# mastbaum/sxmc

Hardware: AMD Instinct MI355X
Metric: NLL evals/sec (10^8 samples, 3 obs, 12 signals) + experiments/sec at 1/2/4/8 GPUs (higher is better)
Workload: dtype f64 exact; f32-on-u16-codes filter decides the unambiguous samples

## Files before the change

### sxmc_amd/csrc/fill_kernels.inc.h

```cpp
#pragma once

#include "sxmc_device_types.h"

#pragma clang fp contract(off)

#ifndef SXMC_MEASURE
#define SXMC_MEASURE 0
#endif

namespace sxfill {

__device__ __forceinline__ constexpr unsigned sx_dbg(unsigned dbg_arg) { return SXMC_MEASURE ? dbg_arg : 0u; }

template <int N>
struct IntC {
  static constexpr int value = N;
  constexpr operator int() const { return N; }
};
template <unsigned long... I>
struct ISeq {};
template <int N, unsigned long... I>
struct MakeISeq : MakeISeq<N - 1, (unsigned long)(N - 1), I...> {};
template <unsigned long... I>
struct MakeISeq<0, I...> {
// ... 107 lines not shown
        pw[q] = 1.0;
        pl[q] = 0.0;
      }
      for (int i = 0; i < npars; i++) {
        const double c = readlane_d(coef, cstart + i);
#pragma unroll
        for (int q = 0; q < SXMC_VEC; q++) {
          p[q] = p[q] + c * pw[q];
          pow_step(pw[q], pl[q], f[K][q]);
        }
      }
    }
    apply_transform<NSLOT>(f, type, f[K], extra_slot, p);
  });
}

constexpr unsigned sx_op(int type, int obs_slot, int extra_slot = 0, int npars = 0) {
  return (unsigned)type | ((unsigned)obs_slot << 4) | ((unsigned)extra_slot << 8) | ((unsigned)npars << 12);
}
constexpr int sx_op_npars(unsigned w) { return ((w >> 12) & 15u) ? (int)((w >> 12) & 15u) : 1; }
template <unsigned... OPS>
constexpr int sx_prog_ncoef() {
  constexpr unsigned ops[] = {OPS..., 0u};
  int c = 0;
  for (int k = 0; k < (int)sizeof...(OPS); k++) c += sx_op_npars(ops[k]);
  return c;
}
template <unsigned... OPS>
constexpr int sx_prog_cstart(int i) {
  constexpr unsigned ops[] = {OPS..., 0u};
  int c = 0;
  for (int k = 0; k < i; k++) c += sx_op_npars(ops[k]);
  return c;
}
template <unsigned... OPS>
struct StaticProg {
  static constexpr bool dynamic = false;
  static constexpr int n = (int)sizeof...(OPS);
  static constexpr int ncoef = sx_prog_ncoef<OPS...>();
  static constexpr unsigned touched = (0u | ... | (1u << ((OPS >> 4) & 15u)));
};
struct DynamicProg {
  static constexpr bool dynamic = true;
  static constexpr int n = 0;
  static constexpr int ncoef = 0;
  static constexpr unsigned touched = ~0u;
};

template <int NSLOT, unsigned OPC>
__device__ __forceinline__ void apply_static(double (&f)[NSLOT][SXMC_VEC], const double* c) {
  constexpr int type = (int)(OPC & 15u), K = (int)((OPC >> 4) & 15u), E = (int)((OPC >> 8) & 15u);
  constexpr int NP = sx_op_npars(OPC);
  static_assert(K < NSLOT && E < NSLOT, "slot out of range");
#pragma unroll
  for (int q = 0; q < SXMC_VEC; q++) {
    double pc = 0.0 + c[0] * 1.0;
    if constexpr (NP > 1) {
      double pw = 1.0 * f[K][q], pl = 0.0;
#pragma unroll
      for (int i = 1; i < NP; i++) {
        pc = pc + c[i] * pw;
        pow_step(pw, pl, f[K][q]);
      }
    }
    if constexpr (type == SXMC_SYST_SHIFT) f[K][q] = f[K][q] + pc;
    if constexpr (type == SXMC_SYST_SCALE) f[K][q] = f[K][q] * (1 + pc);
    if constexpr (type == SXMC_SYST_CTSCALE) f[K][q] = 1 + (f[K][q] - 1) * (1 + pc);
    if constexpr (type == SXMC_SYST_RESOLUTION_SCALE) f[K][q] = f[K][q] + (pc * (f[K][q] - f[E][q]));
  }
}

template <int NSLOT, unsigned... OPS, unsigned long... I>
__device__ __forceinline__ void run_static(double (&f)[NSLOT][SXMC_VEC], const double* c, StaticProg<OPS...>,
                                           ISeq<I...>) {
  (apply_static<NSLOT, OPS>(f, c + sx_prog_cstart<OPS...>((int)I)), ...);
}

typedef float vfloat4 __attribute__((ext_vector_type(4)));

#ifndef SXMC_WG_STAMPS
#define SXMC_WG_STAMPS 0
#endif
#if SXMC_WG_STAMPS && !defined(__HIPCC_RTC__)
extern "C" __device__ unsigned long long sx_wg_stamps[3 * 4096];
#define SX_WG_STAMP(which)                                                                      \
  do {                                                                                          \
    if (threadIdx.x == 0 && blockIdx.x < 4096u) {                                               \
      sx_wg_stamps[(which)*4096 + blockIdx.x] = __builtin_amdgcn_s_memrealtime();               \
    }                                                                                           \
  } while (0)
#else
#define SX_WG_STAMP(which) \
  do {                     \
  } while (0)
#endif
#ifndef SXMC_CACHED_LOADS
#define SXMC_CACHED_LOADS 0
#endif
template <typename T>
__device__ __forceinline__ T stream_load(gptr<const T> p) {
  if constexpr (SXMC_CACHED_LOADS) return *p;
  else return __builtin_nontemporal_load(p);
}

typedef unsigned vuint2 __attribute__((ext_vector_type(2)));

__device__ __forceinline__ void sparse_lookup(const SxSignalDesc& d, gptr<unsigned> counters, unsigned bin) {
  const unsigned mask = (1u << (32 - d.sparse_table_shift)) - 1u;
  unsigned hp = (bin * 0x85EBCA6Bu) >> d.sparse_table_shift;
  for (unsigned probe = 0; probe <= mask; probe++) {
    const vuint2 e = to_global(reinterpret_cast<const vuint2*>(d.sparse_table))[hp];
    if (e[0] == bin) {
      __hip_atomic_fetch_add(&counters[e[1]], 1u, __ATOMIC_RELAXED, __HIP_MEMORY_SCOPE_AGENT);
      return;
    }
    if (e[0] == 0xFFFFFFFFu) return;
    hp = (hp + 1u) & mask;
  }
}

__device__ __forceinline__ void sparse_count(const SxSignalDesc& d, gptr<unsigned> counters, unsigned bin) {
  const unsigned hb = (bin * 0x9E3779B1u) >> d.sparse_filter_shift;
  if (!((to_global(d.sparse_filter)[hb >> 5] >> (hb & 31u)) & 1u)) return;
  sparse_lookup(d, counters, bin);
}

constexpr int kPreGranule = 3;
template <int PREW> struct PreVec { typedef unsigned type; };
template <> struct PreVec<2> { typedef unsigned type __attribute__((ext_vector_type(2))); };
template <> struct PreVec<4> { typedef unsigned type __attribute__((ext_vector_type(4))); };

template <int NSLOT, int PREW>
struct Columns {
  vfloat4 v[NSLOT];
  typename PreVec<PREW>::type pre;
};

template <int NOBS, int PREW, typename PROG>
constexpr bool slot_loaded(int k) {
  return PREW == 0 || PREW == kPreGranule || k >= NOBS || ((PROG::touched >> k) & 1u);
}

template <int PREW>
__device__ __forceinline__ unsigned pre_value(const typename PreVec<PREW>::type& p, int q) {
  if constexpr (PREW == 1) return (p >> (8 * q)) & 0xFFu;
  if constexpr (PREW == 2) return (p[q >> 1] >> (16 * (q & 1))) & 0xFFFFu;
  if constexpr (PREW == 4) return p[q];
  if constexpr (PREW == kPreGranule) return p;
  return 0u;
}
template <int PREW>
constexpr unsigned pre_sentinel() {
  return PREW == 1 ? 0xFFu : PREW == 2 ? 0xFFFFu : 0xFFFFFFFFu;
}

template <int NOBS, int NSLOT, int PREW, typename PROG>
__device__ __forceinline__ void load_columns(Columns<NSLOT, PREW>& c, const gptr<const vfloat4> (&col)[NSLOT],
                                             gptr<const typename PreVec<PREW>::type> pre, unsigned long long v) {
#pragma unroll
  for (int k = 0; k < NSLOT; k++) {
    if constexpr (true) {
      if (slot_loaded<NOBS, PREW, PROG>(k)) {
        c.v[k] = stream_load<vfloat4>(&col[k][v]);
        __builtin_amdgcn_sched_barrier(0);
      }
    }
  }
  if constexpr (PREW == kPreGranule) {
    c.pre = pre[v >> 6];
    __builtin_amdgcn_sched_barrier(0);
  } else if constexpr (PREW != 0) {
    c.pre = stream_load<typename PreVec<PREW>::type>(&pre[v]);
    __builtin_amdgcn_sched_barrier(0);
  }
}

// ... 1483 lines not shown
        unsigned n = 0u;
        for (unsigned r = 0; r < R; r++) n += hist[(unsigned)c * cstride + r * rstride + w];
        total += n;
        if (n != 0u) __hip_atomic_fetch_add(&gbins[lds_slot(w)], n, __ATOMIC_RELAXED, __HIP_MEMORY_SCOPE_AGENT);
      }
      if (use_q) {
#pragma unroll
        for (int off = kWave / 2; off > 0; off >>= 1) total += __shfl_down(total, off, kWave);
        if (lane == 0 && total != 0u) {
          __hip_atomic_fetch_add(&s_norm[c], total, __ATOMIC_RELAXED, __HIP_MEMORY_SCOPE_WORKGROUP);
        }
        __syncthreads();
      }
      if (LDS_HIST && more) {
        __syncthreads();
        for (unsigned b = 4u * tid; b < cstride; b += 4u * nthreads) {
          *reinterpret_cast<vuint4g*>(&hist[(unsigned)c * cstride + b]) = vuint4g{0u, 0u, 0u, 0u};
        }
      }
      if (tid == 0) {
        const unsigned n = s_norm[c];
        if (n != 0u) __hip_atomic_fetch_add(to_global(dc.norm), n, __ATOMIC_RELAXED, __HIP_MEMORY_SCOPE_AGENT);
        s_norm[c] = 0u;
      }
    }
    __syncthreads();
    lds_clean = true;
  }
  SX_WG_STAMP(2);
}

template <unsigned OPC, int XT>
__device__ __forceinline__ void apply_box_interval(double& xl, double& xh, double tl, double th, bool& fin, const double* c) {
  constexpr int type = (int)(OPC & 15u), E = (int)((OPC >> 8) & 15u);
  static_assert(sx_op_npars(OPC) == 1, "not a one-coefficient systematic");
  const double pc = 0.0 + c[0] * 1.0;
  if constexpr (type == SXMC_SYST_SHIFT) {
    xl = xl + pc;
    xh = xh + pc;
  }
  if constexpr (type == SXMC_SYST_SCALE) {
    const double s = 1 + pc, a = xl * s, b = xh * s;
    xl = s >= 0.0 ? a : b;
    xh = s >= 0.0 ? b : a;
  }
  if constexpr (type == SXMC_SYST_CTSCALE) {
    const double s = 1 + pc, a = 1 + (xl - 1) * s, b = 1 + (xh - 1) * s;
    xl = s >= 0.0 ? a : b;
    xh = s >= 0.0 ? b : a;
  }
  if constexpr (type == SXMC_SYST_RESOLUTION_SCALE) {
    static_assert(E == XT, "the boxed observable reads one truth field");
    const double dl = xl - th, dh = xh - tl;
    const double a = pc * dl, b = pc * dh;
    const double ml = pc >= 0.0 ? a : b, mh = pc >= 0.0 ? b : a;
    fin = fin && (__builtin_fabs(dl) < __builtin_inf()) && (__builtin_fabs(dh) < __builtin_inf()) &&
          (__builtin_fabs(ml) < __builtin_inf()) && (__builtin_fabs(mh) < __builtin_inf());
    xl = xl + ml;
    xh = xh + mh;
  }
  fin = fin && (__builtin_fabs(xl) < __builtin_inf()) && (__builtin_fabs(xh) < __builtin_inf());
}
template <int BX, int XT, unsigned... OPS, unsigned long... I>
__device__ __forceinline__ void run_box_interval(double& xl, double& xh, double tl, double th, bool& fin, const double* c,
                                                 StaticProg<OPS...>, ISeq<I...>) {
  ([&] {
    if constexpr ((int)((OPS >> 4) & 15u) == BX) apply_box_interval<OPS, XT>(xl, xh, tl, th, fin, c + sx_prog_cstart<OPS...>((int)I));
  }(), ...);
}
template <int BX, int XT, unsigned... OPS>
constexpr bool prog_is_boxable(StaticProg<OPS...>) {
  return (true && ... &&
          (sx_op_npars(OPS) == 1 && (int)((OPS >> 4) & 15u) != XT &&
           ((int)(OPS & 15u) != SXMC_SYST_RESOLUTION_SCALE ||
            ((int)((OPS >> 4) & 15u) == BX && (int)((OPS >> 8) & 15u) == XT))));
}

#ifndef SXMC_BOX_DRAIN
#define SXMC_BOX_DRAIN 2
#endif
#ifndef SXMC_BOX_GQ
#define SXMC_BOX_GQ 0
#endif
#ifndef SXMC_BOX_PREFETCH
#define SXMC_BOX_PREFETCH 0
#endif
template <int NOBS, int NSLOT, typename PROG>
__device__ __forceinline__ void fill_boxed_body(const SxSignalDesc* __restrict__ descs, const SxSegment* __restrict__ segs,
                                                const unsigned* __restrict__ blk_off, unsigned layout, unsigned dbg_arg) {
  const unsigned dbg = sx_dbg(dbg_arg);
  static_assert(!PROG::dynamic && NOBS == 1 && NSLOT == 3, "one streamed observable, one truth field, the boxed observable");
  constexpr int BX = 2, XT = 1;
  static_assert(prog_is_boxable<BX, XT>(PROG{}), "not a program the boxed form can run");
  constexpr int NC = PROG::ncoef > 0 ? PROG::ncoef : 1;
#ifndef SXMC_BOX_RING
#define SXMC_BOX_RING 8
#endif
  constexpr int kRing = SXMC_BOX_RING;
  constexpr int kDrain = SXMC_BOX_DRAIN;
  static_assert(64 % kRing == 0, "a block of 64 units is a whole number of rounds of the ring");
  typedef typename MakeISeq<PROG::n>::type Seq;
  extern __shared__ unsigned lds[];
  const unsigned tid = threadIdx.x;
  const unsigned nthreads = blockDim.x;
  const unsigned lane = tid & (kWave - 1);
  unsigned* s_norm = lds;
  unsigned* hist = lds + 4;
  const unsigned rstride = layout & 0xFFFFFFu, rlog = (layout >> 24) & 7u, R = 1u << rlog;
  const unsigned cstride = rstride << rlog;
  const unsigned myrep = (lane & (R - 1u)) * rstride;
  const unsigned qlog = layout >> 28;
  const unsigned qwave = qlog ? (1u << qlog) / (nthreads / kWave) : 0u;
  const unsigned gq_min = (unsigned)kRing + 1u;
  const unsigned gq_cap = qwave / 2u > gq_min ? qwave / 2u : gq_min, rq_cap = qwave > gq_cap ? qwave - gq_cap : 0u;
  const unsigned gq_drain = (SXMC_BOX_GQ > 0 && (unsigned)SXMC_BOX_GQ + (unsigned)kRing < gq_cap) ? (unsigned)SXMC_BOX_GQ + (unsigned)kRing : gq_cap;
  unsigned* qrows = lds + 4 + cstride + 64 + 4 + (tid / kWave) * (2u * qwave);
  unsigned* qgran = qrows + 2u * rq_cap;

  bool lds_clean = false;
  const unsigned seg_end = blk_off[blockIdx.x + 1];
  for (unsigned si = blk_off[blockIdx.x]; si < seg_end; ++si) {
    const SxSegment& sg = segs[si];
    const SxSignalDesc& d = descs[sg.sig];
    const unsigned long long v0 = sg.v0, v1 = sg.v1, step = sg.step;
    const unsigned B = (unsigned)d.total_nbins;
    double craw[NC];
#pragma unroll
    for (int q = 0; q < PROG::ncoef; q++) craw[q] = to_global(d.params)[(long)d.coef_par[q] * d.param_stride];
    __builtin_amdgcn_sched_barrier(0);

    gptr<const vfloat4> col[NSLOT];
#pragma unroll
    for (int k = 0; k < NSLOT; k++) {
      col[k] = to_global(reinterpret_cast<const vfloat4*>(d.cols + (unsigned long long)d.slot_col[k] * d.col_pitch));
    }
    gptr<const unsigned> precol = to_global(reinterpret_cast<const unsigned*>(d.pre));
    gptr<const vfloat4> boxes = to_global(reinterpret_cast<const vfloat4*>(d.boxes));
    gptr<const vuint2g> qcol = to_global(d.qcol != nullptr ? reinterpret_cast<const vuint2g*>(d.qcol)
                                                           : reinterpret_cast<const vuint2g*>(d.cols));
    const unsigned vfirst32 = (unsigned)(v0 + tid), step32 = (unsigned)step, vlast32 = (unsigned)(v1 - 1);
    const unsigned vwave32 = vfirst32 - lane;
    const unsigned niter32 = (unsigned)((v1 - v0 + step - 1) / step);

    if (!lds_clean) {
      for (unsigned b = tid; b < cstride; b += nthreads) hist[b] = 0u;
      if (tid < 4) s_norm[tid] = 0u;
      __syncthreads();
    }

    const double lo = d.lower[0], hi = d.upper[0], sc = d.scale[0];
    const int st = d.bin_stride[0];
    const unsigned nbk = (unsigned)d.nbins[0];
    const double olo = d.lower[NOBS], ohi = d.upper[NOBS], osc = d.scale[NOBS];
    const int ost = d.bin_stride[NOBS];
    int stv = st, ostv = ost;
    asm volatile("" : "+v"(stv));
    asm volatile("" : "+v"(ostv));
    const unsigned s_in = (unsigned)st, s_out = s_in * nbk;
    const unsigned oS = B / nbk, oSp = oS | 1u;
    const float inv_in = 1.0f / (float)s_in, inv_out = 1.0f / (float)s_out;
    auto fdiv = [](unsigned x, float inv) -> unsigned { return (unsigned)(((float)x + 0.5f) * inv); };
    auto hist_word = [&](unsigned bin) -> unsigned {
      const unsigned h = fdiv(bin, inv_out), rem = bin - h * s_out, idx = fdiv(rem, inv_in);
      return (idx + 1u) * oSp + h * s_in + (rem - idx * s_in);
    };

    bool wild = false;
#pragma unroll
    for (int q = 0; q < PROG::ncoef; q++) wild = wild || !(__builtin_fabs(craw[q]) < __builtin_inf());

    float af, gf, thr;
    bool use_q = d.qcol != nullptr && rq_cap >= 8u && !wild;
    {
      AffineForm<1> form[1];
      form[0].a[0] = 1.0;
      form[0].c = 0.0;
      const double wlo = d.qbase[0], whi = d.qbase[0] + 65534.0 * d.qstep[0];
      form[0].mag = __builtin_fmax(__builtin_fabs(wlo), __builtin_fabs(whi));
      run_affine<1, BX>(form, craw, PROG{}, Seq{});
      const double alpha = form[0].a[0] * d.qstep[0] * sc;
      const double sum_abs = __builtin_fabs(alpha);
      double g = form[0].c - lo;
      g = g + form[0].a[0] * (d.qbase[0] + 0.5 * d.qstep[0]);
      g = g * sc;
      const double mu = sum_abs * 65536.0 + __builtin_fabs(g) + (double)nbk + 0.25;
      const double epsq = 0.5 * sum_abs * (1.0 + 0x1p-19);
      const double eps = epsq + mu * 0x1p-21 + (form[0].mag + __builtin_fabs(lo)) * sc * 0x1p-44;
      const bool ok = eps < 0.125;
      const double e = eps * 1.01, slack = 0x1p-23;
      af = uniform_f((float)alpha);
      gf = uniform_f((float)(g + e));
      thr = uniform_f((float)(2.0 * e + slack));
      use_q = use_q && (uniform_i(ok ? 1 : 0) != 0);
    }

    unsigned vcnt = 0u;
    unsigned nrow = 0u, ngran = 0u;

    unsigned gword = kOrdSkip, greal = 0u;
    vfloat4 bx_next;
    unsigned pre_next;
    auto meta_load = [&](unsigned it) {
      unsigned vg = vwave32 + (it + lane) * step32;
      vg = vg <= vlast32 ? vg : vlast32;
      bx_next = boxes[vg >> 6];
      pre_next = precol[vg >> 6];
    };
    auto granule_meta = [&](unsigned it) {
      unsigned vg = vwave32 + (it + lane) * step32;
      const bool live = vg <= vlast32;
      vg = live ? vg : vlast32;
      if constexpr (!SXMC_BOX_PREFETCH) meta_load(it);
      const vfloat4 bx = bx_next;
      const unsigned pre = pre_next;
      if constexpr (SXMC_BOX_PREFETCH) meta_load(it + 64u);
      double xl = (double)bx.x, xh = (double)bx.y;
      const double tl = (double)bx.z, th = (double)bx.w;
      bool fin = (__builtin_fabs(xl) < __builtin_inf()) && (__builtin_fabs(xh) < __builtin_inf()) &&
                 (__builtin_fabs(tl) < __builtin_inf()) && (__builtin_fabs(th) < __builtin_inf());
      run_box_interval<BX, XT>(xl, xh, tl, th, fin, craw, PROG{}, Seq{});
      const int i0 = (int)((xl - olo) * osc), i1 = (int)((xh - olo) * osc);
      const int e0 = !(xl >= olo) ? -1 : (!(xl < ohi) ? 0x7FFFFFFF : i0);
      const int e1 = !(xh >= olo) ? -1 : (!(xh < ohi) ? 0x7FFFFFFF : i1);
      const unsigned off = (pre & 0xFFFFFFu) + (unsigned)e0 * (unsigned)ost;
      const unsigned h = fdiv(off, inv_out), rem = off - h * s_out;
      const bool canon = off < (1u << 22) && rem < s_in && (h + 1u) * s_out <= B;
      const bool mixed = !use_q || !fin || e0 != e1 || !canon;
      const bool skip = fin && e0 == e1 && (e0 < 0 || e0 == 0x7FFFFFFF);
      gword = !live ? kOrdSkip : skip ? kOrdSkip : mixed ? kOrdMixed : h * s_in + rem;
      greal = off;
    };

    auto push_granule = [&](unsigned it) {
      if (lane == 0) qgran[2u * ngran] = vwave32 + it * step32;
      ngran += 1u;
    };
    auto push_rows = [&](unsigned rare, unsigned v, unsigned real_off) -> bool {
      unsigned long long mask[SXMC_VEC];
      unsigned total = 0u;
#pragma unroll
      for (int q = 0; q < SXMC_VEC; q++) {
        mask[q] = __builtin_amdgcn_ballot_w64(((rare >> q) & 1u) != 0u);
        total += (unsigned)__builtin_popcountll(mask[q]);
      }
      if (nrow + total > rq_cap) return false;
#pragma unroll
      for (int q = 0; q < SXMC_VEC; q++) {
        if (mask[q] == 0ull) continue;
        const unsigned below = __builtin_amdgcn_mbcnt_hi((unsigned)(mask[q] >> 32),
                                                         __builtin_amdgcn_mbcnt_lo((unsigned)mask[q], 0u));
        if ((rare >> q) & 1u) {
          const unsigned pos = nrow + below;
          qrows[2u * pos] = v * SXMC_VEC + (unsigned)q;
          qrows[2u * pos + 1u] = real_off;
        }
        nrow += (unsigned)__builtin_popcountll(mask[q]);
      }
      return true;
    };

    const int oS4 = (int)(4u * oSp);
    const int oclamp = (dbg & 4u) ? -1 : (int)nbk;
    auto coarse_unit = [&](const vuint2g& w, unsigned it, unsigned v, unsigned word0) {
      int base4 = (int)(4u * (4u + myrep + word0) + 4u * oSp);
      asm volatile("" : "+v"(base4));
      const float c0 = (float)(w.x & 0xFFFFu), c1 = (float)(w.x >> 16), c2 = (float)(w.y & 0xFFFFu), c3 = (float)(w.y >> 16);
      const vfloat2 a2 = {af, af}, g2 = {gf, gf};
      const vfloat2 u01 = __builtin_elementwise_fma(a2, vfloat2{c0, c1}, g2);
      const vfloat2 u23 = __builtin_elementwise_fma(a2, vfloat2{c2, c3}, g2);
      const float us[SXMC_VEC] = {u01.x, u01.y, u23.x, u23.y};
      int addr[SXMC_VEC];
      bool amb[SXMC_VEC];
#pragma unroll
      for (int q = 0; q < SXMC_VEC; q++) {
        const float u = us[q];
        amb[q] = !(__builtin_amdgcn_fractf(u) >= thr);
        int idx;
        asm("v_cvt_flr_i32_f32 %0, %1" : "=v"(idx) : "v"(u));
        int ie;
        asm("v_med3_i32 %0, %1, -1, %2" : "=v"(ie) : "v"(amb[q] ? -1 : idx), "s"(oclamp));
        addr[q] = mad24(ie, oS4, base4);
      }
      const float cmax = __builtin_fmaxf(__builtin_fmaxf(c0, c1), __builtin_fmaxf(c2, c3));
      const bool special = cmax >= (float)SXMC_QCODE_EXACT;
      const bool anyamb = (amb[0] | amb[1]) | (amb[2] | amb[3]);
      if (__builtin_amdgcn_ballot_w64(anyamb || special) != 0ull) {
        const float cs[SXMC_VEC] = {c0, c1, c2, c3};
        unsigned rare = 0u;
#pragma unroll
        for (int q = 0; q < SXMC_VEC; q++) {
          rare |= amb[q] ? (1u << q) : 0u;
          if (cs[q] >= (float)SXMC_QCODE_EXACT) {
            addr[q] = base4 - oS4;
            rare = cs[q] >= (float)SXMC_QCODE_NEVER ? (rare & ~(1u << q)) : (rare | (1u << q));
          }
        }
        const unsigned real_off = (unsigned)__builtin_amdgcn_readlane((int)greal, (int)(it & 63u));
        if (!push_rows(rare, v, real_off)) {
          push_granule(it);
          return;
        }
      }
      if (dbg & 32u) {
        vcnt += (unsigned)(addr[0] ^ addr[1] ^ addr[2] ^ addr[3]) == 12345u ? 1u : 0u;
        return;
      }
#pragma unroll
      for (int q = 0; q < SXMC_VEC; q++) {
        unsigned* wp = reinterpret_cast<unsigned*>(reinterpret_cast<char*>(lds) + addr[q]);
        __hip_atomic_fetch_add(wp, 1u, __ATOMIC_RELAXED, __HIP_MEMORY_SCOPE_WORKGROUP);
      }
    };

    auto count_exact = [&](bool ind, int bin) {
      vcnt += (ind && !((unsigned)bin < B)) ? 1u : 0u;
      if (ind && ((unsigned)bin < B)) {
        __hip_atomic_fetch_add(&hist[myrep + hist_word((unsigned)bin)], 1u, __ATOMIC_RELAXED, __HIP_MEMORY_SCOPE_WORKGROUP);
      }
    };
    auto drain = [&]() {
      if (dbg & 16u) nrow = ngran = 0u;
      vfloat4 rawf[kDrain][NSLOT];
      unsigned prew[kDrain];
      auto load_granule = [&](int s, unsigned g) {
        const unsigned vw = (unsigned)uniform_i((int)qgran[2u * g]);
        const unsigned vc = vw + lane < vlast32 ? vw + lane : vlast32;
#pragma unroll
        for (int k = 0; k < NSLOT; k++) rawf[s][k] = __builtin_nontemporal_load(&col[k][vc]);
        prew[s] = precol[vc >> 6];
      };
      unsigned row = 0u, w1 = 0u;
      float rowf = 0.0f;
      if (lane < nrow) {
        row = qrows[2u * lane];
        w1 = qrows[2u * lane + 1u];
        rowf = ((gptr<const float>)col[0])[row];
      }
#pragma unroll
      for (int s = 0; s < kDrain; s++) {
        if ((unsigned)s < ngran) load_granule(s, (unsigned)s);
      }
      for (unsigned i0 = 0; i0 < nrow; i0 += kWave) {
        if (i0 != 0u && i0 + lane < nrow) {
          row = qrows[2u * (i0 + lane)];
          w1 = qrows[2u * (i0 + lane) + 1u];
          rowf = ((gptr<const float>)col[0])[row];
        }
        if (i0 + lane < nrow) {
          double f[NSLOT][SXMC_VEC];
#pragma unroll
          for (int k = 0; k < NSLOT; k++) f[k][0] = f[k][1] = f[k][2] = f[k][3] = 0.0;
          f[0][0] = f[0][1] = f[0][2] = f[0][3] = (double)rowf;
          run_static_part<NSLOT, BX, false>(f, craw, PROG{}, Seq{});
          const double x = f[0][0];
          const bool ind = (x >= lo) & (x < hi);
          const int idx = (int)((x - lo) * sc);
          count_exact(ind, mad24(idx, stv, (int)w1));
        }
      }
      for (unsigned g0 = 0; g0 < ngran; g0 += (unsigned)kDrain) {
        if (g0 != 0u) {
#pragma unroll
          for (int s = 0; s < kDrain; s++) {
            if (g0 + (unsigned)s < ngran) load_granule(s, g0 + (unsigned)s);
          }
        }
#pragma unroll
        for (int s = 0; s < kDrain; s++) {
          if (g0 + (unsigned)s >= ngran) break;
          const unsigned off = (unsigned)uniform_i((int)prew[s]) & 0xFFFFFFu;
          double f[NSLOT][SXMC_VEC];
#pragma unroll
          for (int k = 0; k < NSLOT; k++) {
            f[k][0] = (double)rawf[s][k].x;
            f[k][1] = (double)rawf[s][k].y;
            f[k][2] = (double)rawf[s][k].z;
            f[k][3] = (double)rawf[s][k].w;
          }
          run_static<NSLOT>(f, craw, PROG{}, Seq{});
#pragma unroll
          for (int q = 0; q < SXMC_VEC; q++) {
            const double x = f[0][q], y = f[BX][q];
            const bool ind = (x >= lo) & (x < hi) & (y >= olo) & (y < ohi);
            const int idx = (int)((x - lo) * sc), oidx = (int)((y - olo) * osc);
            count_exact(ind, mad24(oidx, ostv, mad24(idx, stv, (int)off)));
          }
        }
      }
      nrow = ngran = 0u;
    };

    vuint2g rq[kRing];
    const unsigned vfirst8 = vfirst32 * 8u, vlast8 = vlast32 * 8u, step8 = step32 * 8u;
    auto issue = [&](int slot, unsigned it) {
      unsigned o = vfirst8 + it * step8;
      o = o < vlast8 ? o : vlast8;
      rq[slot] = __builtin_nontemporal_load((gptr<const vuint2g>)((gptr<const char>)qcol + (unsigned long long)o));
      __builtin_amdgcn_sched_barrier(0);
    };
    const unsigned climit = (unsigned)uniform_i((int)oS);
    {
      unsigned it = 0u;
      if constexpr (SXMC_BOX_PREFETCH) meta_load(0u);
#pragma unroll
      for (int i = 0; i < kRing; i++) issue(i, (unsigned)i);
      while (it < niter32) {
        if ((it & 63u) == 0u) granule_meta(it);
        const unsigned block_end = niter32 < (it | 63u) + 1u ? niter32 : (it | 63u) + 1u;
        bool full = false;
        while (it < block_end && !full) {
#pragma unroll
          for (int i = 0; i < kRing; i++) {
#pragma unroll
            for (int e = 0; e < 2; e++) asm volatile("" : "+v"(rq[i][e]));
            const unsigned iu = it + (unsigned)i;
            if (iu < block_end) {
              const unsigned word0 = (unsigned)__builtin_amdgcn_readlane((int)gword, (int)(iu & 63u));
              if (dbg & 1u) {
                vcnt += (rq[i].x == 12345u && word0 == 77u) ? 1u : 0u;
              } else if (word0 < climit) coarse_unit(rq[i], iu, vfirst32 + iu * step32, word0);
              else if (word0 == kOrdMixed) push_granule(iu);
            }
            issue(i, iu + (unsigned)kRing);
          }
          it = block_end - it < (unsigned)kRing ? block_end : it + (unsigned)kRing;
          full = ngran + (unsigned)kRing > gq_drain;
        }
        if (full) {
          drain();
          __builtin_amdgcn_s_waitcnt(0);
        }
      }
    }
    drain();

    {
      unsigned t = vcnt;
#pragma unroll
      for (int off = kWave / 2; off > 0; off >>= 1) t += __shfl_down(t, off, kWave);
      if (lane == 0 && t != 0u) __hip_atomic_fetch_add(&s_norm[0], t, __ATOMIC_RELAXED, __HIP_MEMORY_SCOPE_WORKGROUP);
    }
    __syncthreads();
    {
      gptr<unsigned> gbins = to_global(d.bins);
      const bool more = si + 1u < seg_end;
      const unsigned nwords = nbk * oSp;
      const float invSp = 1.0f / (float)oSp;
      unsigned total = 0u;
#pragma unroll 4
      for (unsigned w = tid; w < nwords; w += nthreads) {
        const unsigned idx = fdiv(w, invSp), r = w - idx * oSp;
        unsigned n = 0u;
        for (unsigned rep = 0; rep < R; rep++) n += hist[rep * rstride + oSp + w];
        if (r < oS) {
          total += n;
          const unsigned h = fdiv(r, inv_in);
          if (n != 0u) {
            __hip_atomic_fetch_add(&gbins[h * s_out + idx * s_in + (r - h * s_in)], n, __ATOMIC_RELAXED, __HIP_MEMORY_SCOPE_AGENT);
          }
        }
      }
#pragma unroll
      for (int off = kWave / 2; off > 0; off >>= 1) total += __shfl_down(total, off, kWave);
      if (lane == 0 && total != 0u) __hip_atomic_fetch_add(&s_norm[0], total, __ATOMIC_RELAXED, __HIP_MEMORY_SCOPE_WORKGROUP);
      __syncthreads();
      if (more) {
        for (unsigned b = 4u * tid; b < cstride; b += 4u * nthreads) {
          *reinterpret_cast<vuint4g*>(&hist[b]) = vuint4g{0u, 0u, 0u, 0u};
        }
      }
      if (tid == 0) {
        const unsigned n = s_norm[0];
        if (n != 0u) __hip_atomic_fetch_add(to_global(d.norm), n, __ATOMIC_RELAXED, __HIP_MEMORY_SCOPE_AGENT);
        s_norm[0] = 0u;
      }
    }
    __syncthreads();
    lds_clean = true;
  }
}

template <int NOBS, int NSLOT, bool LDS_HIST, typename PROG, int PREW>
__global__ __launch_bounds__(1024) void fill_kernel(const SxSignalDesc* __restrict__ descs,
                                                    const SxSegment* __restrict__ segs,
                                                    const unsigned* __restrict__ blk_off, unsigned hist_words,
                                                    unsigned dbg) {
  fill_body<NOBS, NSLOT, LDS_HIST, PROG, PREW>(descs, segs, blk_off, hist_words, dbg);
}

template <int NOBS, int NSLOT, typename PROG>
__global__ __launch_bounds__(1024) void fill_sparse_kernel(const SxSignalDesc* __restrict__ descs,
                                                           const SxSegment* __restrict__ segs,
                                                           const unsigned* __restrict__ blk_off, unsigned smax,
                                                           unsigned dbg) {
  fill_sparse_body<NOBS, NSLOT, PROG>(descs, segs, blk_off, smax, dbg);
}

#ifndef SXMC_ORDERED_BOUND
#define SXMC_ORDERED_BOUND 1024
#endif
template <int NOBS, int NSLOT, typename PROG, bool LDS_HIST = true>
__global__ __launch_bounds__(SXMC_ORDERED_BOUND) void fill_ordered_kernel(const SxSignalDesc* __restrict__ descs,
                                                            const SxSegment* __restrict__ segs,
                                                            const unsigned* __restrict__ blk_off, unsigned layout,
                                                            unsigned dbg) {
  SxChainDescs one;
  one.d[0] = one.d[1] = one.d[2] = one.d[3] = descs;
  fill_ordered_body<NOBS, NSLOT, PROG, 1, LDS_HIST>(one, segs, blk_off, layout, dbg);
}

template <int NOBS, int NSLOT, typename PROG>
__global__ __launch_bounds__(SXMC_ORDERED_BOUND) void fill_boxed_kernel(const SxSignalDesc* __restrict__ descs,
                                                          const SxSegment* __restrict__ segs,
                                                          const unsigned* __restrict__ blk_off, unsigned layout,
                                                          unsigned dbg) {
  fill_boxed_body<NOBS, NSLOT, PROG>(descs, segs, blk_off, layout, dbg);
}

}
```

### sxmc_amd/csrc/pdfz_kernels.hip

```cpp
#include <hip/hip_runtime.h>
#include <hip/hip_ext.h>

#include <cstring>
#include <vector>

#include "nll_device.h"

#include "fill_kernels.inc.h"

#pragma clang fp contract(off)

namespace {

using namespace sxfill;


__global__ __launch_bounds__(256) void zero_kernel(const SxSignalDesc* __restrict__ descs, unsigned* ticket) {
  const SxSignalDesc& d = descs[blockIdx.y];
  unsigned* bins = d.bins;
  const unsigned n = (unsigned)d.total_nbins;
  const unsigned n4 = n >> 2;
  uint4* b4 = reinterpret_cast<uint4*>(bins);
  const unsigned stride = gridDim.x * blockDim.x;
  for (unsigned i = blockIdx.x * blockDim.x + threadIdx.x; i < n4; i += stride) {
// ... 640 lines not shown
      sxdev::peek_next_proposal_device(a.nparameters, a.rng, a.jump_width, a.v_current, v_b);
    } else {
      collect();
    }
    __syncthreads();
    for (int j = threadIdx.x; j < nsig; j += blockDim.x) {
      *hist_a[j].norm = 0u;
      *hist_b[j].norm = 0u;
    }
    return;
  }
  const bool second = blockIdx.x >= nvb;
  const unsigned vb = second ? blockIdx.x - nvb : blockIdx.x;
  const double t = eval_nll_block_part(second ? lookup_b : lookup_a, nsig, npoints, second ? weight_b : weight_a,
                                       second ? v_b : a.v_proposed, a.nexpected, a.n_mc, a.source_id,
                                       second ? norms_b : a.norms, sh, vb, nvb);
  __shared__ int s_clear;
  if (threadIdx.x == 0) {
    __hip_atomic_store(slots + blockIdx.x, isnan(t) ? kSlotNaN : (unsigned long long)__double_as_longlong(t),
                       __ATOMIC_RELAXED, __HIP_MEMORY_SCOPE_AGENT);
    asm volatile("s_waitcnt vmcnt(0)" ::: "memory");
    unsigned it = 0;
    for (; it < kEndSpinLimit; it++) {
      if (__hip_atomic_load(slots + blockIdx.x, __ATOMIC_RELAXED, __HIP_MEMORY_SCOPE_AGENT) == kSlotEmpty) break;
      __builtin_amdgcn_s_sleep(1);
    }
    if (it == kEndSpinLimit) __hip_atomic_fetch_add(timeouts, 1u, __ATOMIC_RELAXED, __HIP_MEMORY_SCOPE_AGENT);
    s_clear = it < kEndSpinLimit ? 1 : 0;
  }
  __syncthreads();
  if (!s_clear) return;
  const unsigned npieces = 2u * zblocks * (unsigned)nsig;
  for (unsigned p = blockIdx.x; p < npieces; p += W) {
    const unsigned which = p / (zblocks * (unsigned)nsig);
    const unsigned q = p - which * zblocks * (unsigned)nsig;
    const SxSignalDesc& d = (which ? hist_b : hist_a)[q / zblocks];
    const unsigned chunk = q % zblocks;
    unsigned* bins = d.bins;
    const unsigned n = (unsigned)d.total_nbins;
    const unsigned n4 = n >> 2;
    uint4* b4 = reinterpret_cast<uint4*>(bins);
    const unsigned stride = zblocks * blockDim.x;
    for (unsigned i = chunk * blockDim.x + threadIdx.x; i < n4; i += stride) b4[i] = make_uint4(0u, 0u, 0u, 0u);
    if (chunk == 0 && threadIdx.x < (n & 3u)) bins[(n4 << 2) + threadIdx.x] = 0u;
  }
}

__global__ __launch_bounds__(256) void eval_nll_chains_kernel(SxChainEnds e, int nsig) {
  extern __shared__ double sh[];
  const SxChainEnd& c = e.c[blockIdx.y];
  if (blockIdx.x >= c.nblocks) return;
  const double t = eval_nll_block_part(c.lookup_descs, nsig, c.nrows, c.weight, c.a.v_proposed, c.a.nexpected, c.a.n_mc,
                                       c.a.source_id, c.a.norms, sh, blockIdx.x, c.nblocks);
  if (threadIdx.x == 0 && !isnan(t)) c.sums[blockIdx.x] = t;
}

__global__ __launch_bounds__(256) void finish_zero_chains_kernel(SxChainEnds e, int nsig, unsigned zblocks) {
  const SxChainEnd& c = e.c[blockIdx.y];
  const SxStepArgs& a = c.a;
  if (blockIdx.x == 0) {
    sxdev::finish_step_device(c.nblocks, c.sums, a.nsignals, a.nsources, a.means, a.sigmas, a.rng, a.nll_current,
                              a.nll_proposed, a.v_current, a.v_proposed, a.accepted, a.counter, a.jump_buffer,
                              a.nparameters, a.jump_width, a.nexpected, a.n_mc, a.source_id, a.norms,
                              a.debug_mode != 0);
    __syncthreads();
    for (int j = threadIdx.x; j < nsig; j += blockDim.x) *c.hist_descs[j].norm = 0u;
    if (threadIdx.x == 0 && c.ticket) *c.ticket = 0u;
    return;
  }
  const unsigned b = blockIdx.x - 1u;
  const SxSignalDesc& d = c.hist_descs[b / zblocks];
  const unsigned chunk = b % zblocks;
  unsigned* bins = d.bins;
  const unsigned n = (unsigned)d.total_nbins;
  const unsigned n4 = n >> 2;
  uint4* b4 = reinterpret_cast<uint4*>(bins);
  const unsigned stride = zblocks * blockDim.x;
  for (unsigned i = chunk * blockDim.x + threadIdx.x; i < n4; i += stride) b4[i] = make_uint4(0u, 0u, 0u, 0u);
  if (chunk == 0 && threadIdx.x < (n & 3u)) bins[(n4 << 2) + threadIdx.x] = 0u;
}

#if SXMC_WG_STAMPS
extern "C" {
__device__ unsigned long long sx_wg_stamps[3 * 4096];
}
extern "C" int sxmc_debug_read_wg_stamps(unsigned long long* out, int n) {
  return (int)hipMemcpyFromSymbol(out, HIP_SYMBOL(sx_wg_stamps), sizeof(unsigned long long) * (size_t)n);
}
#endif

__global__ __launch_bounds__(256) void prebin_kernel(const SxSignalDesc* __restrict__ dp, unsigned mask, int width,
                                                     void* out) {
  const SxSignalDesc& d = *dp;
  const unsigned long long npad = d.nvec * SXMC_VEC;
  const unsigned sentinel = width == 1 ? 0xFFu : width == 2 ? 0xFFFFu : 0xFFFFFFFFu;
  const unsigned long long step = (unsigned long long)gridDim.x * blockDim.x;
  for (unsigned long long i = (unsigned long long)blockIdx.x * blockDim.x + threadIdx.x; i < npad; i += step) {
    unsigned val = sentinel;
    if (i < d.nsamples) {
      bool ok = true;
      int part = 0;
      for (int k = 0; k < d.nobs; k++) {
        if (!((mask >> k) & 1u)) continue;
        const double x = (double)to_global(d.cols)[(unsigned long long)k * d.col_pitch + i];
        ok = ok && (x >= d.lower[k]) && (x < d.upper[k]);
        part += (int)((x - d.lower[k]) * d.scale[k]) * d.bin_stride[k];
      }
      if (ok) val = (unsigned)part;
    }
    if (width == 1) static_cast<unsigned char*>(out)[i] = (unsigned char)val;
    else if (width == 2) static_cast<unsigned short*>(out)[i] = (unsigned short)val;
    else static_cast<unsigned*>(out)[i] = val;
  }
}

#if SXMC_MEASURE
__global__ void pow_int_kernel(const double* __restrict__ x, int n, int i, double* __restrict__ out) {
  for (int k = blockIdx.x * blockDim.x + threadIdx.x; k < n; k += gridDim.x * blockDim.x) {
    double h = 1.0, l = 0.0;
    for (int t = 0; t < i; t++) pow_step(h, l, x[k]);
    out[k] = h;
  }
}
#endif

__global__ __launch_bounds__(256) void transpose_kernel(const float* __restrict__ aos, float* __restrict__ cols,
                                                        unsigned long long n, int F,
                                                        unsigned long long pitch) {
  const unsigned long long npad = (n + SXMC_VEC - 1) / SXMC_VEC * SXMC_VEC;
  const unsigned long long step = (unsigned long long)gridDim.x * blockDim.x;
  for (unsigned long long i = (unsigned long long)blockIdx.x * blockDim.x + threadIdx.x; i < npad; i += step) {
    for (int k = 0; k < F; k++) {
      cols[(unsigned long long)k * pitch + i] = (i < n) ? aos[i * F + k] : __int_as_float(0x7fc00000);
    }
  }
}

__global__ __launch_bounds__(256) void untranspose_obs_kernel(const float* __restrict__ cols, float* __restrict__ out,
                                                              unsigned long long n, int nobs,
                                                              unsigned long long pitch, float dataset) {
  const unsigned long long step = (unsigned long long)gridDim.x * blockDim.x;
  for (unsigned long long i = (unsigned long long)blockIdx.x * blockDim.x + threadIdx.x; i < n; i += step) {
    for (int k = 0; k < nobs; k++) out[i * (nobs + 1) + k] = cols[(unsigned long long)k * pitch + i];
    out[i * (nobs + 1) + nobs] = dataset;
  }
}

template <typename K, typename... A>
void launch_fill(const SxLaunchShape& sh, K k, dim3 grid, dim3 block, size_t lds, hipStream_t s, A... args) {
  if (sh.ev_start && sh.ev_stop) {
    hipExtLaunchKernelGGL(k, grid, block, (std::uint32_t)lds, s, (hipEvent_t)sh.ev_start, (hipEvent_t)sh.ev_stop, 0u,
                          args...);
  } else {
    hipLaunchKernelGGL(k, grid, block, lds, s, args...);
  }
}

template <bool LDS_HIST, typename PROG, int PREW>
constexpr bool has_step_form() {
  return LDS_HIST && PROG::n == 0 && (PREW == 1 || PREW == 2);
}

template <int NOBS, int NSLOT, bool LDS_HIST, typename PROG, int PREW = 0>
hipError_t launch_fill_k(const SxLaunchShape& sh, const SxSignalDesc* descs, const SxSegment* segs,
                         const unsigned* blk_off, hipStream_t s) {
  const unsigned hist_words = (unsigned)(sh.lds_bytes / 4 - 4 - (LDS_HIST ? 64 : 0));
  if constexpr (has_step_form<LDS_HIST, PROG, PREW>()) {
    if (sh.tail) {
      auto ks = fill_step_kernel<NOBS, NSLOT, PROG, PREW>;
      if (sh.lds_bytes > 48 * 1024) {
// ... 492 lines not shown
```

Before: 12970.

## Share final granule drain across waves and hoist ring/meta prefetch before LDS clear

The first quantized-code ring loads and the first two box/prebin metadata loads are now issued before the LDS histogram clear and its barrier, so their latency overlaps the clear. The LDS clear uses 128-bit stores. The final drain after the streaming loop is shared across the workgroup: each wave publishes its granule count, a prefix scan assigns granules round-robin to all waves, and per-wave queues are read across slices, which balances the tail work. Under a debug flag it also adds per-workgroup timing and max/add stamp instrumentation. The shared drain adds a __syncthreads and cross-wave LDS indexing.

```diff
diff --git a/sxmc_amd/csrc/fill_kernels.inc.h b/sxmc_amd/csrc/fill_kernels.inc.h
--- a/sxmc_amd/csrc/fill_kernels.inc.h
+++ b/sxmc_amd/csrc/fill_kernels.inc.h
@@ -213,16 +213,36 @@
 #define SXMC_WG_STAMPS 0
 #endif
 #if SXMC_WG_STAMPS && !defined(__HIPCC_RTC__)
-extern "C" __device__ unsigned long long sx_wg_stamps[3 * 4096];
+extern "C" __device__ unsigned long long sx_wg_stamps[8 * 4096];
 #define SX_WG_STAMP(which)                                                                      \
   do {                                                                                          \
     if (threadIdx.x == 0 && blockIdx.x < 4096u) {                                               \
       sx_wg_stamps[(which)*4096 + blockIdx.x] = __builtin_amdgcn_s_memrealtime();               \
     }                                                                                           \
   } while (0)
+#define SX_WG_STAMP_MAX(which, value)                                                                                      \
+  do {                                                                                                                     \
+    if ((threadIdx.x & 63u) == 0u && blockIdx.x < 4096u) {                                                                 \
+      __hip_atomic_fetch_max(&sx_wg_stamps[(which)*4096 + blockIdx.x], (unsigned long long)(value), __ATOMIC_RELAXED,      \
+                             __HIP_MEMORY_SCOPE_AGENT);                                                                    \
+    }                                                                                                                      \
+  } while (0)
+#define SX_WG_STAMP_ADD(which, value)                                                                                      \
+  do {                                                                                                                     \
+    if ((threadIdx.x & 63u) == 0u && blockIdx.x < 4096u) {                                                                 \
+      __hip_atomic_fetch_add(&sx_wg_stamps[(which)*4096 + blockIdx.x], (unsigned long long)(value), __ATOMIC_RELAXED,      \
+                             __HIP_MEMORY_SCOPE_AGENT);                                                                    \
+    }                                                                                                                      \
+  } while (0)
 #else
 #define SX_WG_STAMP(which) \
   do {                     \
+  } while (0)
+#define SX_WG_STAMP_MAX(which, value) \
+  do {                                \
+  } while (0)
+#define SX_WG_STAMP_ADD(which, value) \
+  do {                                \
   } while (0)
 #endif
 #ifndef SXMC_CACHED_LOADS
@@ -1872,9 +1892,6 @@
 #ifndef SXMC_BOX_GQ
 #define SXMC_BOX_GQ 0
 #endif
-#ifndef SXMC_BOX_PREFETCH
-#define SXMC_BOX_PREFETCH 0
-#endif
 template <int NOBS, int NSLOT, typename PROG>
 __device__ __forceinline__ void fill_boxed_body(const SxSignalDesc* __restrict__ descs, const SxSegment* __restrict__ segs,
                                                 const unsigned* __restrict__ blk_off, unsigned layout, unsigned dbg_arg) {
@@ -1908,6 +1925,7 @@
   unsigned* qgran = qrows + 2u * rq_cap;
 
   bool lds_clean = false;
+  SX_WG_STAMP(0);
   const unsigned seg_end = blk_off[blockIdx.x + 1];
   for (unsigned si = blk_off[blockIdx.x]; si < seg_end; ++si) {
     const SxSegment& sg = segs[si];
@@ -1932,8 +1950,33 @@
     const unsigned vwave32 = vfirst32 - lane;
     const unsigned niter32 = (unsigned)((v1 - v0 + step - 1) / step);
 
+    vfloat4 bx_first[2];
+    unsigned pre_first[2];
+    auto meta_load = [&](unsigned it, vfloat4& bx, unsigned& pre) {
+      unsigned vg = vwave32 + (it + lane) * step32;
+      vg = vg <= vlast32 ? vg : vlast32;
+      bx = boxes[vg >> 6];
+      pre = precol[vg >> 6];
+    };
+    vuint2g rq[kRing];
+    const unsigned vfirst8 = vfirst32 * 8u, vlast8 = vlast32 * 8u, step8 = step32 * 8u;
+    auto issue = [&](int slot, unsigned it) {
+      unsigned o = vfirst8 + it * step8;
+      o = o < vlast8 ? o : vlast8;
+      rq[slot] = __builtin_nontemporal_load((gptr<const vuint2g>)((gptr<const char>)qcol + (unsigned long long)o));
+      __builtin_amdgcn_sched_barrier(0);
+    };
+    meta_load(0u, bx_first[0], pre_first[0]);
+    meta_load(64u, bx_first[1], pre_first[1]);
+    __builtin_amdgcn_sched_barrier(0);
+#pragma unroll
+    for (int i = 0; i < kRing; i++) issue(i, (unsigned)i);
+    if (!lds_clean) SX_WG_STAMP(1);
+
     if (!lds_clean) {
-      for (unsigned b = tid; b < cstride; b += nthreads) hist[b] = 0u;
+      for (unsigned b = 4u * tid; b < cstride; b += 4u * nthreads) {
+        *reinterpret_cast<vuint4g*>(&hist[b]) = vuint4g{0u, 0u, 0u, 0u};
+      }
       if (tid < 4) s_norm[tid] = 0u;
       __syncthreads();
     }
@@ -1988,22 +2031,19 @@
     unsigned nrow = 0u, ngran = 0u;
 
     unsigned gword = kOrdSkip, greal = 0u;
-    vfloat4 bx_next;
-    unsigned pre_next;
-    auto meta_load = [&](unsigned it) {
-      unsigned vg = vwave32 + (it + lane) * step32;
-      vg = vg <= vlast32 ? vg : vlast32;
-      bx_next = boxes[vg >> 6];
-      pre_next = precol[vg >> 6];
-    };
     auto granule_meta = [&](unsigned it) {
-      unsigned vg = vwave32 + (it + lane) * step32;
-      const bool live = vg <= vlast32;
-      vg = live ? vg : vlast32;
-      if constexpr (!SXMC_BOX_PREFETCH) meta_load(it);
-      const vfloat4 bx = bx_next;
-      const unsigned pre = pre_next;
-      if constexpr (SXMC_BOX_PREFETCH) meta_load(it + 64u);
+      const bool live = vwave32 + (it + lane) * step32 <= vlast32;
+      vfloat4 bx;
+      unsigned pre;
+      if (it == 0u) {
+        bx = bx_first[0];
+        pre = pre_first[0];
+      } else if (it == 64u) {
+        bx = bx_first[1];
+        pre = pre_first[1];
+      } else {
+        meta_load(it, bx, pre);
+      }
       double xl = (double)bx.x, xh = (double)bx.y;
       const double tl = (double)bx.z, th = (double)bx.w;
       bool fin = (__builtin_fabs(xl) < __builtin_inf()) && (__builtin_fabs(xh) < __builtin_inf()) &&
@@ -2108,12 +2148,25 @@
         __hip_atomic_fetch_add(&hist[myrep + hist_word((unsigned)bin)], 1u, __ATOMIC_RELAXED, __HIP_MEMORY_SCOPE_WORKGROUP);
       }
     };
-    auto drain = [&]() {
+    auto drain = [&](const bool shared) {
       if (dbg & 16u) nrow = ngran = 0u;
       vfloat4 rawf[kDrain][NSLOT];
       unsigned prew[kDrain];
+      if (shared && lane == 0) qgran[1] = ngran;
+      unsigned wcnt = 0u, wincl = 0u;
+      unsigned gfirst = 0u, gstep = (unsigned)kDrain, gtotal = ngran;
+      const unsigned qslice = 2u * qwave;
+      const unsigned* qall = qgran - (tid / kWave) * qslice;
       auto load_granule = [&](int s, unsigned g) {
-        const unsigned vw = (unsigned)uniform_i((int)qgran[2u * g]);
+        unsigned entry;
+        if (shared) {
+          const unsigned wv = (unsigned)__builtin_popcountll(__builtin_amdgcn_ballot_w64(lane < 16u && wincl <= g));
+          const unsigned before = (unsigned)__builtin_amdgcn_readlane((int)(wincl - wcnt), (int)wv);
+          entry = qall[wv * qslice + 2u * (g - before)];
+        } else {
+          entry = qgran[2u * g];
+        }
+        const unsigned vw = (unsigned)uniform_i((int)entry);
         const unsigned vc = vw + lane < vlast32 ? vw + lane : vlast32;
 #pragma unroll
         for (int k = 0; k < NSLOT; k++) rawf[s][k] = __builtin_nontemporal_load(&col[k][vc]);
@@ -2126,9 +2179,11 @@
         w1 = qrows[2u * lane + 1u];
         rowf = ((gptr<const float>)col[0])[row];
       }
-#pragma unroll
-      for (int s = 0; s < kDrain; s++) {
-        if ((unsigned)s < ngran) load_granule(s, (unsigned)s);
+      if (!shared) {
+#pragma unroll
+        for (int s = 0; s < kDrain; s++) {
+          if ((unsigned)s < ngran) load_granule(s, (unsigned)s);
+        }
       }
       for (unsigned i0 = 0; i0 < nrow; i0 += kWave) {
         if (i0 != 0u && i0 + lane < nrow) {
@@ -2148,16 +2203,30 @@
           count_exact(ind, mad24(idx, stv, (int)w1));
         }
       }
-      for (unsigned g0 = 0; g0 < ngran; g0 += (unsigned)kDrain) {
-        if (g0 != 0u) {
+      if (shared) {
+        __syncthreads();
+        const unsigned nwaves = nthreads / kWave;
+        wcnt = lane < nwaves ? qall[lane * qslice + 1u] : 0u;
+        wincl = wcnt;
+#pragma unroll
+        for (int off = 1; off < 16; off <<= 1) {
+          const unsigned below = __shfl_up(wincl, off, kWave);
+          wincl += lane >= (unsigned)off ? below : 0u;
+        }
+        gtotal = (unsigned)__builtin_amdgcn_readlane((int)wincl, 15);
+        gfirst = (tid / kWave) * (unsigned)kDrain;
+        gstep = nwaves * (unsigned)kDrain;
+      }
+      for (unsigned g0 = gfirst; g0 < gtotal; g0 += gstep) {
+        if (shared || g0 != 0u) {
 #pragma unroll
           for (int s = 0; s < kDrain; s++) {
-            if (g0 + (unsigned)s < ngran) load_granule(s, g0 + (unsigned)s);
+            if (g0 + (unsigned)s < gtotal) load_granule(s, g0 + (unsigned)s);
           }
         }
 #pragma unroll
         for (int s = 0; s < kDrain; s++) {
-          if (g0 + (unsigned)s >= ngran) break;
+          if (g0 + (unsigned)s >= gtotal) break;
           const unsigned off = (unsigned)uniform_i((int)prew[s]) & 0xFFFFFFu;
           double f[NSLOT][SXMC_VEC];
 #pragma unroll
@@ -2180,20 +2249,9 @@
       nrow = ngran = 0u;
     };
 
-    vuint2g rq[kRing];
-    const unsigned vfirst8 = vfirst32 * 8u, vlast8 = vlast32 * 8u, step8 = step32 * 8u;
-    auto issue = [&](int slot, unsigned it) {
-      unsigned o = vfirst8 + it * step8;
-      o = o < vlast8 ? o : vlast8;
-      rq[slot] = __builtin_nontemporal_load((gptr<const vuint2g>)((gptr<const char>)qcol + (unsigned long long)o));
-      __builtin_amdgcn_sched_barrier(0);
-    };
     const unsigned climit = (unsigned)uniform_i((int)oS);
     {
       unsigned it = 0u;
-      if constexpr (SXMC_BOX_PREFETCH) meta_load(0u);
-#pragma unroll
-      for (int i = 0; i < kRing; i++) issue(i, (unsigned)i);
       while (it < niter32) {
         if ((it & 63u) == 0u) granule_meta(it);
         const unsigned block_end = niter32 < (it | 63u) + 1u ? niter32 : (it | 63u) + 1u;
@@ -2217,12 +2275,19 @@
           full = ngran + (unsigned)kRing > gq_drain;
         }
         if (full) {
-          drain();
+          drain(false);
           __builtin_amdgcn_s_waitcnt(0);
         }
       }
     }
-    drain();
+#if SXMC_WG_STAMPS
+    SX_WG_STAMP_MAX(2, ~__builtin_amdgcn_s_memrealtime());
+    SX_WG_STAMP_MAX(3, __builtin_amdgcn_s_memrealtime());
+    SX_WG_STAMP_MAX(6, ngran);
+    SX_WG_STAMP_ADD(7, ngran);
+#endif
+    drain(true);
+    SX_WG_STAMP_MAX(4, __builtin_amdgcn_s_memrealtime());
 
     {
       unsigned t = vcnt;
@@ -2268,6 +2333,7 @@
     __syncthreads();
     lds_clean = true;
   }
+  SX_WG_STAMP(5);
 }
 
 template <int NOBS, int NSLOT, bool LDS_HIST, typename PROG, int PREW>
diff --git a/sxmc_amd/csrc/pdfz_kernels.hip b/sxmc_amd/csrc/pdfz_kernels.hip
--- a/sxmc_amd/csrc/pdfz_kernels.hip
+++ b/sxmc_amd/csrc/pdfz_kernels.hip
@@ -746,10 +746,16 @@
 
 #if SXMC_WG_STAMPS
 extern "C" {
-__device__ unsigned long long sx_wg_stamps[3 * 4096];
+__device__ unsigned long long sx_wg_stamps[8 * 4096];
 }
 extern "C" int sxmc_debug_read_wg_stamps(unsigned long long* out, int n) {
   return (int)hipMemcpyFromSymbol(out, HIP_SYMBOL(sx_wg_stamps), sizeof(unsigned long long) * (size_t)n);
+}
+extern "C" int sxmc_debug_clear_wg_stamps(void) {
+  void* p = nullptr;
+  hipError_t e = hipGetSymbolAddress(&p, HIP_SYMBOL(sx_wg_stamps));
+  if (e == hipSuccess) e = hipMemset(p, 0, sizeof(unsigned long long) * 8 * 4096);
+  return (int)e;
 }
 #endif
 
```

Result: no change. 12770, median of 2 (-1.5%).
